# jeff-regier/Celeste.jl

Hardware: AMD Instinct MI355X
Metric: sources/sec (ELBO value+gradient+Hessian+KL per target source) (higher is better)
Workload: dtype f64; 1 GPU; BASELINE.json configs[2]: synthetic 2048x1489x5 SDSS-size field, 2000 star+galaxy sources, fp64, Sa=1 with value-only neighbours, psf_K=2; gather_backend=none, neighbor_links_rank0=3526

## Files before the change

### celeste.jl_amd/csrc/celeste_abi.hip

```cpp
#include <hip/hip_runtime.h>
#include <algorithm>
#include <atomic>
#include <cmath>
#include <cstdio>
#include <cstdlib>
#include <cstring>
#include <mutex>
#include <unordered_map>
#include <vector>

#include "elbo_kernels.h"
#include "optim_kernels.h"
#include "fused_kernels.h"
#include "host_tables.h"

struct celeste_group;

#define EVAL_FUSED_MAX 32

#define HIP_TRY(expr)                                                                    \
    do {                                                                                 \
        hipError_t e__ = (expr);                                                         \
        if (e__ != hipSuccess) {                                                         \
            fprintf(stderr, "celeste_mi355x: %s failed: %s (%s:%d)\n", #expr,            \
// ... 50 lines not shown
    return cap;
}
static hipError_t staging_alloc(void **p, size_t bytes) {
    *p = nullptr;
    int k = -1;
    if (pinned_pool_cap() && bytes <= (1u << 20)) { k = 0; while (((size_t)4096 << k) < bytes) ++k; }
    if (k < 0) return hipHostMalloc(p, std::max<size_t>(bytes, 1), hipHostMallocPortable);
    PinnedPool &pp = pinned_pool();
    {
        std::lock_guard<std::mutex> lk(pp.mu);
        if (!pp.idle[k].empty()) { *p = pp.idle[k].back(); pp.idle[k].pop_back(); pp.idle_bytes -= (size_t)4096 << k; pp.live[*p] = k; return hipSuccess; }
    }
    hipError_t e = hipHostMalloc(p, (size_t)4096 << k, hipHostMallocPortable);
    if (e == hipSuccess) { std::lock_guard<std::mutex> lk(pp.mu); pp.live[*p] = k; }
    return e;
}
static void staging_free(void *p) {
    if (!p) return;
    {
        PinnedPool &pp = pinned_pool();
        std::lock_guard<std::mutex> lk(pp.mu);
        auto it = pp.live.find(p);
        if (it != pp.live.end()) {
            const int k = it->second;
            pp.live.erase(it);
            if (pp.idle_bytes + ((size_t)4096 << k) <= pinned_pool_cap()) { pp.idle[k].push_back(p); pp.idle_bytes += (size_t)4096 << k; return; }
        }
    }
    (void)hipHostFree(p);
}


struct celeste_images {
    int device = 0;
    int N = 0;
    std::vector<DevImage> h_images;
    std::vector<void *> plane_allocs;
    DevImage *d_images = nullptr;
    std::atomic<int> refs{1};
};

static void images_release(celeste_images *im) {
    if (!im || im->refs.fetch_sub(1) != 1) return;
    (void)hipSetDevice(im->device);
    for (void *p : im->plane_allocs) (void)hipFree(p);
    if (im->d_images) (void)hipFree(im->d_images);
    delete im;
}

struct celeste_ctx {
    int device = 0;
    celeste_images *imgs = nullptr;
    hipStream_t stream = nullptr;
    hipStream_t copy_stream = nullptr;
    bool copy_stream_checked = false;
    int N = 0, S = 0, K = 0, NC = 0, n_stamps = 0;
    int chunk_px = 256, CH = 1;
    int max_npx = 0;
    std::vector<DevPatch> h_patches;
    std::vector<int64_t> h_nbr_off;
    std::vector<int32_t> h_nbr_idx;
    DevImage *d_images = nullptr;
    DevPatch *d_patches = nullptr;
    double *d_coefs = nullptr;
    float *d_coefs_f = nullptr;
    uint8_t *d_bitmaps = nullptr;
    int64_t *d_nbr_off = nullptr;
    int32_t *d_nbr_idx = nullptr;
    PriorDev *d_prior = nullptr;
    SrcImg *d_srcimg = nullptr;
    Comp *d_comps = nullptr;
    SrcGeo *d_geo = nullptr;
    int64_t *d_val_off = nullptr;
    double2 *d_val = nullptr;
    int32_t *d_needed = nullptr;
    int32_t stamp = 0;
    std::vector<int32_t> h_vis_off, h_vis_img, h_vis_src;
    int32_t *d_vis_off = nullptr, *d_vis_img = nullptr, *d_vis_src = nullptr;
    int4 *d_value_items = nullptr;
    int4 *d_vitems_src = nullptr;
    int32_t *d_vitem_off = nullptr;
    std::vector<int32_t> h_vitem_off;
    int64_t n_value_items = 0;
    int32_t *d_prep_mark = nullptr;
    double *d_lg_sum = nullptr;
    int64_t *d_nv_base = nullptr;
    int32_t *d_nbr_vis = nullptr;
    int2 *d_items = nullptr;
    size_t items_cap = 0;
    std::vector<int32_t> h_src_chunks;
    std::vector<int64_t> h_top_chunks;
    int max_src_chunks = 0;
    int32_t *d_work = nullptr, *d_work_blk = nullptr, *d_work_total = nullptr;
    size_t work_cap = 0, work_blk_cap = 0;
    int M = 1;
    bool dense = false;
    int64_t V = 0;
    std::vector<int64_t> h_tile_off;
    int64_t *d_tile_off = nullptr;
    int64_t n_tiles = 0;
    int sum_tiles = 4, RCH = 1;
    double *d_rec = nullptr;
    double *d_acc_split = nullptr;
    size_t acc_split_cap = 0;
    double *d_acc = nullptr;
    size_t acc_cap = 0;
    int32_t *d_rec_off = nullptr;
    size_t rec_off_cap = 0;
    double *d_vp = nullptr;
    int32_t *d_targets = nullptr;
    double *d_v = nullptr, *d_d = nullptr, *d_h = nullptr;
    int64_t *d_cnt = nullptr;
    int32_t *d_status = nullptr;
    size_t stage_cap = 0;
    double *p_vp = nullptr;
    int32_t *p_targets = nullptr, *p_status = nullptr;
    double *p_v = nullptr, *p_d = nullptr, *p_h = nullptr;
    int64_t *p_cnt = nullptr;
    size_t pin_cap = 0;
    double *d_small_in = nullptr, *p_small_in = nullptr, *d_small_out = nullptr, *p_small_out = nullptr;
    static const int MAX_PARTS = 8;
    hipEvent_t part_done[MAX_PARTS] = {}, part_copied[MAX_PARTS] = {};
    struct OptBuffers {
        size_t cap = 0;
        double *d_vp = nullptr, *d_v = nullptr, *d_d = nullptr, *d_h = nullptr, *d_H = nullptr, *d_T = nullptr, *d_S = nullptr, *d_pos = nullptr;
        int32_t *d_targets = nullptr, *d_act[2] = {nullptr, nullptr}, *d_evt[2] = {nullptr, nullptr}, *d_count = nullptr,
                *d_st = nullptr;
        void *d_state = nullptr;
        static const int RING = 4;
        double *h_vp = nullptr;
        void *h_state = nullptr;
        int32_t *h_count = nullptr;
        hipEvent_t ev[RING] = {};
    } opt;
    struct FusedBuffers {
        size_t cap_t = 0, cap_rec = 0, cap_q = 0, cap_saved = 0;
        bool arrivals_dirty = true;
        int4 *d_chunk_desc = nullptr;
        int2 *d_tgt_rec = nullptr;
        int32_t *d_q_items = nullptr, *d_q_ctl = nullptr, *d_arrivals = nullptr;
        double *d_saved = nullptr;
        int32_t *h_ctl = nullptr;
        int max_resident = 0;
        int cus = 0;
    } fused;
    struct Scratch { void *p = nullptr; size_t cap = 0; } scratch[24];
    int timing = 0;
    hipEvent_t ev[5] = {nullptr, nullptr, nullptr, nullptr, nullptr};
    int ev_split = 0;
    int ev_valid = 0;
};

#define ABI_CATCH catch (const std::bad_alloc &) { return CELESTE_ERR_ALLOC; } catch (...) { return CELESTE_ERR_HIP; }

extern "C" int celeste_version(void) { return CELESTE_ABI_VERSION; }

extern "C" const char *celeste_strerror(int status) {
    switch (status) {
        case CELESTE_OK: return "ok";
        case CELESTE_ERR_INVALID_ARG: return "invalid argument";
        case CELESTE_ERR_NONFINITE_INPUT: return "vp contains NaNs or Infs";
        case CELESTE_ERR_NONFINITE_RESULT: return "ELBO value, gradient or Hessian contains Inf/NaNs";
        case CELESTE_ERR_HIP: return "HIP runtime error";
        case CELESTE_ERR_NO_DEVICE: return "no HIP device (the engine has no CPU fallback)";
        case CELESTE_ERR_ALLOC: return "allocation failed";
        case CELESTE_ERR_ABORTED: return "device group aborted: a member failed in front of a collective (destroy the group and create it again)";
// ... 249 lines not shown
        PriorDev pd;
        pd.p = pr->prior ? *pr->prior : DEFAULT_PRIOR;
        for (int i = 0; i < 2; ++i) for (int d = 0; d < 8; ++d) inv4_logdet(pd.p.color_cov[i][d], pd.inv_cov[i][d], &pd.logdet[i][d]);
        CTX_TRY(dev_upload(&c->d_prior, &pd, 1));
    }
    {
        static std::mutex consts_mu;
        static bool consts_ready[16] = {};
        std::lock_guard<std::mutex> lk(consts_mu);
        if (device < 0 || device >= 16 || !consts_ready[device]) {
            double eta[16], nu[16];
            galaxy_prototypes(eta, nu);
            if (hipMemcpyToSymbol(HIP_SYMBOL(c_eta), eta, sizeof eta) != hipSuccess ||
                hipMemcpyToSymbol(HIP_SYMBOL(c_nu), nu, sizeof nu) != hipSuccess) {
                celeste_ctx_destroy(c); return CELESTE_ERR_HIP;
            }
            hipLaunchKernelGGL(exp_table_kernel, dim3(1), dim3(64), 0, nullptr);
            if (hipStreamSynchronize(nullptr) != hipSuccess) { celeste_ctx_destroy(c); return CELESTE_ERR_HIP; }
            if (device >= 0 && device < 16) consts_ready[device] = true;
        }
    }
    CTX_TRY(dev_upload<SrcImg>(&c->d_srcimg, nullptr, (size_t)c->V));
    CTX_TRY(dev_upload<Comp>(&c->d_comps, nullptr, (size_t)c->V * c->NC));
    CTX_TRY(dev_upload<SrcGeo>(&c->d_geo, nullptr, (size_t)c->S));
    {
        std::vector<int64_t> voff(c->h_patches.size());
        int64_t tot = 0;
        for (size_t q = 0; q < c->h_patches.size(); ++q) { voff[q] = tot; tot += (int64_t)c->h_patches[q].H2 * c->h_patches[q].W2; }
        CTX_TRY(dev_upload(&c->d_val_off, voff.data(), voff.size()));
        CTX_TRY(dev_upload<double2>(&c->d_val, nullptr, (size_t)tot));
        CTX_TRY(dev_upload<int32_t>(&c->d_needed, nullptr, (size_t)c->S));
        if (hipMemset(c->d_needed, 0, (size_t)c->S * sizeof(int32_t)) != hipSuccess) { celeste_ctx_destroy(c); return CELESTE_ERR_HIP; }
    }

    CTX_TRY(dev_upload(&c->d_vis_off, c->h_vis_off.data(), c->h_vis_off.size()));
    CTX_TRY(dev_upload(&c->d_vis_img, c->h_vis_img.data(), c->h_vis_img.size()));
    CTX_TRY(dev_upload(&c->d_vis_src, c->h_vis_src.data(), c->h_vis_src.size()));
    CTX_TRY(dev_upload<double>(&c->d_lg_sum, nullptr, (size_t)c->V));
    if (c->V > 0)
        hipLaunchKernelGGL(patch_lgamma_kernel, dim3((unsigned)c->V), dim3(256), 0, nullptr, c->d_images, c->d_patches,
                           c->d_vis_img, c->d_bitmaps, c->d_lg_sum);
    const char *env_chunk = getenv("CELESTE_CHUNK_PX");
    if (env_chunk && atoi(env_chunk) >= 64) c->chunk_px = (atoi(env_chunk) + 63) / 64 * 64;
    c->CH = c->max_npx > 0 ? (c->max_npx + c->chunk_px - 1) / c->chunk_px : 1;
    c->h_src_chunks.assign((size_t)c->S, 0);
    for (int s = 0; s < c->S; ++s) {
        for (int v = c->h_vis_off[s]; v < c->h_vis_off[s + 1]; ++v) {
            const DevPatch &q = c->h_patches[v];
            c->h_src_chunks[s] += (q.H2 * q.W2 + c->chunk_px - 1) / c->chunk_px;
        }
        c->max_src_chunks = std::max(c->max_src_chunks, c->h_src_chunks[s]);
    }
    auto hv = [c](int s, int n) -> int64_t {
        if (c->dense) return (int64_t)s * c->N + n;
        const int32_t *b = c->h_vis_img.data() + c->h_vis_off[s], *e = c->h_vis_img.data() + c->h_vis_off[s + 1];
        const int32_t *it = std::lower_bound(b, e, n);
        return it != e && *it == n ? (int64_t)(it - c->h_vis_img.data()) : -1;
    };
    if (!c->dense) {
        std::vector<int64_t> base((size_t)c->S + 1, 0);
        for (int s = 0; s < c->S; ++s)
            base[s + 1] = base[s] + (int64_t)(c->h_vis_off[s + 1] - c->h_vis_off[s]) * (c->h_nbr_off[s + 1] - c->h_nbr_off[s]);
        std::vector<int32_t> nv((size_t)base[c->S]);
        for (int s = 0; s < c->S; ++s) {
            const int64_t K = c->h_nbr_off[s + 1] - c->h_nbr_off[s];
            for (int v = c->h_vis_off[s]; v < c->h_vis_off[s + 1]; ++v)
                for (int64_t q = 0; q < K; ++q)
                    nv[base[s] + (int64_t)(v - c->h_vis_off[s]) * K + q] = (int32_t)hv(c->h_nbr_idx[c->h_nbr_off[s] + q], c->h_vis_img[v]);
        }
        CTX_TRY(dev_upload(&c->d_nv_base, base.data(), base.size()));
        CTX_TRY(dev_upload(&c->d_nbr_vis, nv.data(), nv.size()));
    }
    {
        std::vector<int32_t> sorted(c->h_src_chunks);
        std::sort(sorted.begin(), sorted.end(), [](int32_t a, int32_t b) { return a > b; });
        c->h_top_chunks.assign((size_t)c->S + 1, 0);
        for (int s = 0; s < c->S; ++s) c->h_top_chunks[s + 1] = c->h_top_chunks[s] + sorted[s];
    }
    CTX_TRY(dev_upload<int32_t>(&c->d_work_total, nullptr, 1));
    {
        if (c->N > 0xffff) { celeste_ctx_destroy(c); return CELESTE_ERR_INVALID_ARG; }
        const int n_cls = c->chunk_px / 64;
        std::vector<std::vector<std::pair<int32_t, int32_t>>> by_len(n_cls);
        for (int s = 0; s < c->S; ++s)
            for (int64_t q = c->h_nbr_off[s]; q < c->h_nbr_off[s + 1]; ++q) {
                const int s2 = c->h_nbr_idx[q];
                for (int va = c->h_vis_off[s]; va < c->h_vis_off[s + 1]; ++va) {
                    const int n = c->h_vis_img[va];
                    const int64_t vb = hv(s2, n);
                    if (vb < 0) continue;
                    const DevPatch &a = c->h_patches[va], &b = c->h_patches[vb];
                    const int rh = std::min(a.off_h + a.H2, b.off_h + b.H2) - std::max(a.off_h, b.off_h);
                    const int rw = std::min(a.off_w + a.W2, b.off_w + b.W2 - 1) - std::max(a.off_w, b.off_w);
                    if (rh <= 0 || rw <= 0) continue;
                    const int npx = rh * rw, nch = (npx + c->chunk_px - 1) / c->chunk_px;
                    for (int ch = 0; ch < nch; ++ch) {
                        const int px = std::min(c->chunk_px, npx - ch * c->chunk_px);
                        by_len[n_cls - (px + 63) / 64].push_back({(int32_t)q, (int32_t)(n | (ch << 16))});
                    }
                }
            }
        std::vector<int32_t> link_src(c->h_nbr_idx.size());
        for (int s = 0; s < c->S; ++s)
            for (int64_t q = c->h_nbr_off[s]; q < c->h_nbr_off[s + 1]; ++q) link_src[q] = s;
        std::vector<int4> desc;
        for (auto &v : by_len)
            for (auto &e : v) {
                const int t = link_src[e.first], s2 = c->h_nbr_idx[e.first], n = e.second & 0xffff, ch = e.second >> 16;
                desc.push_back(make_int4((int)hv(s2, n), (int)hv(t, n), ch, t));
            }
        c->n_value_items = (int64_t)desc.size();
        CTX_TRY(dev_upload(&c->d_value_items, desc.data(), desc.size()));
        c->h_vitem_off.assign((size_t)c->S + 1, 0);
        for (auto &d : desc) c->h_vitem_off[(size_t)d.w + 1]++;
        for (int s = 0; s < c->S; ++s) c->h_vitem_off[s + 1] += c->h_vitem_off[s];
        {
            std::vector<int4> by_src(desc.size());
            std::vector<int32_t> fill(c->h_vitem_off.begin(), c->h_vitem_off.end() - 1);
            for (auto &d : desc) by_src[(size_t)fill[d.w]++] = d;
            CTX_TRY(dev_upload(&c->d_vitems_src, by_src.data(), by_src.size()));
            CTX_TRY(dev_upload(&c->d_vitem_off, c->h_vitem_off.data(), c->h_vitem_off.size()));
        }
        CTX_TRY(dev_upload<int32_t>(&c->d_prep_mark, nullptr, (size_t)c->S));
        if (hipMemset(c->d_prep_mark, 0, (size_t)c->S * sizeof(int32_t)) != hipSuccess) { celeste_ctx_destroy(c); return CELESTE_ERR_HIP; }
    }
    {
        c->h_tile_off.resize(c->h_patches.size());
        int64_t tot = 0;
        for (size_t q = 0; q < c->h_patches.size(); ++q) {
            c->h_tile_off[q] = tot;
            tot += ((int64_t)c->h_patches[q].H2 * c->h_patches[q].W2 + 63) / 64;
        }
        c->n_tiles = tot;
        if (const char *e = getenv("CELESTE_SUM_TILES")) if (atoi(e) > 0) c->sum_tiles = atoi(e);
        c->RCH = std::max(1, ((c->max_npx + 63) / 64 + c->sum_tiles - 1) / c->sum_tiles);
    }
    if (hipStreamSynchronize(nullptr) != hipSuccess) { celeste_ctx_destroy(c); return CELESTE_ERR_HIP; }
#undef CTX_TRY
    *out = c;
    return CELESTE_OK;
} ABI_CATCH

extern "C" void celeste_ctx_destroy(celeste_ctx_t *c) {
    if (!c) return;
    (void)hipSetDevice(c->device);
    if (c->stream) (void)hipStreamSynchronize(c->stream);
    if (c->copy_stream) (void)hipStreamSynchronize(c->copy_stream);
    void *ptrs[] = {c->d_patches, c->d_coefs, c->d_coefs_f, c->d_bitmaps, c->d_nbr_off, c->d_nbr_idx, c->d_prior,
                    c->d_srcimg, c->d_comps, c->d_geo, c->d_val_off, c->d_val, c->d_needed, c->d_vis_off, c->d_vis_img, c->d_vis_src, c->d_value_items, c->d_vitems_src, c->d_vitem_off, c->d_prep_mark, c->d_rec_off, c->d_lg_sum, c->d_nv_base, c->d_nbr_vis, c->d_items, c->d_work, c->d_work_blk, c->d_work_total, c->d_tile_off, c->d_rec, c->d_acc_split, c->d_acc, c->d_vp, c->d_targets, c->d_v, c->d_d, c->d_h,
                    c->d_cnt, c->d_status};
    for (void *p : ptrs) if (p) (void)hipFree(p);
    {
        auto &o = c->opt;
        void *optr[] = {o.d_vp, o.d_v, o.d_d, o.d_h, o.d_H, o.d_T, o.d_S, o.d_pos, o.d_targets, o.d_act[0], o.d_act[1], o.d_evt[0], o.d_evt[1],
                        o.d_count, o.d_st, o.d_state};
        for (void *q : optr) if (q) (void)hipFree(q);
        void *hptr[] = {o.h_vp, o.h_state, o.h_count};
        for (void *q : hptr) if (q) staging_free(q);
        for (int k = 0; k < celeste_ctx::OptBuffers::RING; ++k) if (o.ev[k]) (void)hipEventDestroy(o.ev[k]);
        auto &f = c->fused;
        void *fptr[] = {f.d_chunk_desc, f.d_tgt_rec, f.d_q_items, f.d_q_ctl, f.d_arrivals, f.d_saved};
        for (void *q : fptr) if (q) (void)hipFree(q);
        if (f.h_ctl) staging_free(f.h_ctl);
    }
    for (auto &sc : c->scratch) if (sc.p) (void)hipFree(sc.p);
    for (int i = 0; i < 5; ++i) if (c->ev[i]) (void)hipEventDestroy(c->ev[i]);
    for (int i = 0; i < celeste_ctx::MAX_PARTS; ++i) {
        if (c->part_done[i]) (void)hipEventDestroy(c->part_done[i]);
        if (c->part_copied[i]) (void)hipEventDestroy(c->part_copied[i]);
    }
    void *pins[] = {c->p_vp, c->p_targets, c->p_status, c->p_v, c->p_d, c->p_h, c->p_cnt, c->p_small_in, c->p_small_out};
    if (c->d_small_in) (void)hipFree(c->d_small_in);
    if (c->d_small_out) (void)hipFree(c->d_small_out);
    for (void *q : pins) if (q) staging_free(q);
    stream_retire(c->device, c->stream);
    stream_retire(c->device, c->copy_stream);
    images_release(c->imgs);
    delete c;
}

template <class T>
static hipError_t scratch_get(celeste_ctx_t *c, int k, size_t bytes, T **out) {
    auto &s = c->scratch[k];
    if (bytes > s.cap) {
        hipError_t e = s.p ? hipStreamSynchronize(c->stream) : hipSuccess;
        if (e != hipSuccess) return e;
        if (s.p) { (void)hipFree(s.p); s.p = nullptr; s.cap = 0; }
        e = hipMalloc(&s.p, std::max<size_t>(bytes, 256));
        if (e != hipSuccess) return e;
        s.cap = std::max<size_t>(bytes, 256);
    }
    *out = (T *)s.p;
    return hipSuccess;
}

static int launch_eval(celeste_ctx_t *c, const double *d_vp, int32_t n_targets, const int32_t *d_targets,
                       uint32_t flags, double *d_v, double *d_d, double *d_h, int64_t *d_counters, int32_t *d_status,
                       void *stream_, bool render_neighbors, const int32_t *d_active_rank = nullptr,
                       int64_t n_chunks = -1, bool tables_current = false, const int32_t *d_live = nullptr,
                       bool prep_all = false, bool render_only = false, const int32_t *d_h_pos = nullptr);

extern "C" int celeste_elbo_eval_batch_device(celeste_ctx_t *c, const double *d_vp, int32_t n_targets,
                                              const int32_t *d_targets, uint32_t flags, double *d_v, double *d_d,
                                              double *d_h, int64_t *d_counters, int32_t *d_status, void *stream_) try {
    return launch_eval(c, d_vp, n_targets, d_targets, flags, d_v, d_d, d_h, d_counters, d_status, stream_, true);
} ABI_CATCH

static int ensure_part_events(celeste_ctx_t *c, int n) {
    for (int k = 0; k < n && k < celeste_ctx::MAX_PARTS; ++k) {
        if (!c->part_done[k]) HIP_TRY(hipEventCreateWithFlags(&c->part_done[k], hipEventDisableTiming));
        if (!c->part_copied[k]) HIP_TRY(hipEventCreateWithFlags(&c->part_copied[k], hipEventDisableTiming));
    }
    return CELESTE_OK;
}

static void fused_args_tables(celeste_ctx_t *c, FusedArgs &A) {
    A.images = c->d_images; A.patches = c->d_patches; A.coefs = c->d_coefs; A.bitmaps = c->d_bitmaps;
    A.nbr_off = c->d_nbr_off; A.nbr_idx = c->d_nbr_idx; A.val_off = c->d_val_off; A.val = c->d_val;
    A.nv_base = c->d_nv_base; A.nbr_vis = c->d_nbr_vis; A.items = c->dense ? nullptr : c->d_items; A.geo = c->d_geo;
    A.prior = c->d_prior; A.vis_off = c->d_vis_off; A.vis_img = c->d_vis_img; A.lg_sum = c->d_lg_sum; A.rec_off = c->d_rec_off;
    A.N = c->N; A.NC = c->NC; A.K = c->K; A.M = c->M; A.CH = c->CH; A.chunk_px = c->chunk_px;
    A.acc = c->d_acc;
    A.st = nullptr; A.Hstate = nullptr; A.Tstate = nullptr; A.Spec = nullptr; A.q_items = nullptr; A.q_ctl = nullptr; A.q_cap = 0; A.timeout_ticks = 0;
    A.j_R = 0; A.j_gshift = 0; A.j_dep = nullptr; A.j_succ_off = nullptr; A.j_succ = nullptr; A.j_vitem_off = nullptr;
    A.j_vitems = nullptr; A.j_render_arr = nullptr; A.j_saved = nullptr; A.j_pos = nullptr; A.j_srcimg = nullptr;
    A.j_comps = nullptr; A.j_geo = nullptr;
}

static int fused_buffers(celeste_ctx_t *c, size_t n, size_t rec, hipStream_t stream) {
    auto &fb = c->fused;
    if (n > fb.cap_t) {
        if (fb.d_tgt_rec || fb.d_arrivals) HIP_TRY(hipStreamSynchronize(stream));
// ... 70 lines not shown
    if (eval_fused) G = 1;
    const int n_classes = WORK_CLASSES;
    if ((size_t)n_wblk * (n_classes + 1) > c->work_blk_cap) {
        if (c->d_work_blk) { HIP_TRY(hipStreamSynchronize(stream)); HIP_TRY(hipFree(c->d_work_blk)); c->d_work_blk = nullptr; }
        HIP_TRY(hipMalloc((void **)&c->d_work_blk, (size_t)n_wblk * (n_classes + 1) * sizeof(int32_t)));
        c->work_blk_cap = (size_t)n_wblk * (n_classes + 1);
    }
    const bool derivs = (flags & (CELESTE_FLAG_GRAD | CELESTE_FLAG_HESS)) != 0;
    const bool split = (flags & CELESTE_FLAG_SPLIT) != 0;
    if (split) {
        if (!(flags & CELESTE_FLAG_HESS)) return CELESTE_ERR_INVALID_ARG;
        if (!c->d_rec) {
            HIP_TRY(hipStreamSynchronize(stream));
            if (dev_upload(&c->d_tile_off, c->h_tile_off.data(), c->h_tile_off.size()) != CELESTE_OK) return CELESTE_ERR_HIP;
            if (hipMalloc((void **)&c->d_rec, (size_t)std::max<int64_t>(c->n_tiles, 1) * ACC_N * 64 * sizeof(double)) != hipSuccess)
                return CELESTE_ERR_ALLOC;
        }
        const size_t need_s = (size_t)n_targets * c->M * c->RCH * ACC_N;
        if (need_s > c->acc_split_cap) {
            if (c->d_acc_split) { HIP_TRY(hipStreamSynchronize(stream)); HIP_TRY(hipFree(c->d_acc_split)); c->d_acc_split = nullptr; }
            HIP_TRY(hipMalloc((void **)&c->d_acc_split, need_s * sizeof(double)));
            c->acc_split_cap = need_s;
        }
    }
    if (c->timing) HIP_TRY(hipEventRecord(c->ev[0], stream));
    if (render_neighbors && ++c->stamp == 0x7fffffff) {
        HIP_TRY(hipMemsetAsync(c->d_needed, 0, (size_t)c->S * sizeof(int32_t), stream));
        c->stamp = 1;
    }
    const int geo_S = render_neighbors ? c->S : -1;
    const size_t setup_threads = std::max<size_t>(render_neighbors ? (size_t)c->S : 0, (size_t)n_targets * (c->dense ? 1 : c->M));
    int32_t *const prep_mark = render_neighbors && !tables_current && !prep_all ? c->d_prep_mark : nullptr;
    bool prep_fused = false;
    bool records_described = false;
    if (eval_fused) { int stb = fused_buffers(c, (size_t)n_targets, rec_cap, stream); if (stb != CELESTE_OK) return stb; }
    if (n_visits <= WORK1_MAX_VISITS && !getenv("CELESTE_PARALLEL_WORKLIST")) {
        const unsigned setup_blocks = (unsigned)((setup_threads + WORK1_SETUP - 1) / WORK1_SETUP);
        prep_fused = !render_neighbors && !getenv("CELESTE_NO_FUSED_PREP");
        const bool prep_all_here = render_neighbors && !tables_current && c->V > 0 && c->V <= WORK1_PREP_ALL_MAX &&
                                   (n_targets >= WORK1_PREP_ALL_MIN_TARGETS || c->V <= WORK1_PREP_ALL_TINY) && !getenv("CELESTE_NO_FUSED_PREP");
        const int prep_n = prep_all_here ? (int)c->V : n_visits;
        if (prep_all_here) prep_fused = true;
        const unsigned prep_blocks = prep_fused ? (unsigned)((prep_n + WORK1_NT / 64 - 1) / (WORK1_NT / 64)) : 0u;
        const bool records_described_here = eval_fused && c->dense && !d_live && !getenv("CELESTE_NO_FUSED_DESCRIBE");
        hipLaunchKernelGGL(setup_worklist_kernel, dim3(1 + setup_blocks + prep_blocks), dim3(WORK1_NT),
                           0, stream, d_vp, geo_S, c->d_geo, d_targets, n_targets, c->d_vis_off, c->d_vis_img, c->M,
                           c->dense ? nullptr : c->d_items, render_neighbors ? c->d_needed : nullptr, c->stamp, c->d_patches,
                           c->N, CH, chunk_px, G, (int)c->dense, c->d_work, c->d_work_total, d_live, prep_mark,
                           c->d_nbr_off, c->d_nbr_idx, c->d_rec_off, (int)setup_blocks, c->d_images, c->K, c->d_srcimg,
                           c->d_comps, prep_all_here ? (int)c->V : 0, c->d_vis_src,
                           records_described_here ? c->fused.d_chunk_desc : nullptr, records_described_here ? c->fused.d_tgt_rec : nullptr,
                           c->chunk_px);
        records_described = records_described_here;
    } else {
        hipLaunchKernelGGL(setup_kernel, dim3((unsigned)((setup_threads + 63) / 64)), dim3(64), 0, stream, d_vp, geo_S,
                           c->d_geo, d_targets, n_targets, c->d_vis_off, c->d_vis_img, c->M, c->dense ? nullptr : c->d_items,
                           render_neighbors ? c->d_needed : nullptr, c->stamp, prep_mark, c->d_nbr_off, c->d_nbr_idx, d_live);
        hipLaunchKernelGGL(work_count_kernel, dim3(n_wblk), dim3(WORK_NT), 0, stream, d_targets, n_visits, c->d_patches,
                           c->d_vis_off, c->d_vis_img, c->N, c->M, chunk_px, G, (int)c->dense, c->d_work_blk, d_live);
        hipLaunchKernelGGL(work_scan_kernel, dim3(1), dim3(1024), 0, stream, c->d_work_blk, n_wblk * (n_classes + 1),
                           c->d_work_total, n_wblk * n_classes);
        hipLaunchKernelGGL(work_fill_kernel, dim3(n_wblk), dim3(WORK_NT), 0, stream, d_targets, n_visits, c->d_patches,
                           c->d_vis_off, c->d_vis_img, c->N, c->M, CH, chunk_px, G, (int)c->dense, c->d_work_blk, c->d_work, d_live,
                           c->d_rec_off);
    }
    if (render_neighbors) {
        if (c->V > 0 && !tables_current && !prep_fused)
            hipLaunchKernelGGL(prep_kernel, dim3((unsigned)c->V), dim3(64), 0, stream, d_vp, c->d_images, c->d_patches,
                               c->d_vis_src, c->d_vis_img, c->N, c->K, c->d_srcimg, c->d_comps, nullptr, c->d_vis_off, c->M,
                               (int)c->dense, nullptr, prep_mark, c->stamp);
    } else if (!prep_fused) {
        hipLaunchKernelGGL(prep_kernel, dim3((unsigned)std::max(n_visits, 1)), dim3(64), 0, stream, d_vp, c->d_images,
                           c->d_patches, c->d_vis_src, c->d_vis_img, c->N, c->K, c->d_srcimg, c->d_comps, d_targets,
                           c->d_vis_off, c->M, (int)c->dense, d_live, nullptr, 0);
    }
    if (render_neighbors) {
    if (c->n_value_items > 0)
    {
        const bool wide_items = n_targets <= VALUE_WIDE_MAX && c->chunk_px == 256 && !getenv("CELESTE_NO_WIDE_VALUE");
#define LAUNCH_VALUE(R, WAVES)                                                                                              \
        hipLaunchKernelGGL((value_kernel<R, WAVES>), dim3((unsigned)c->n_value_items), dim3(64 * WAVES), 0, stream,       \
                           c->d_patches, c->d_coefs, c->d_srcimg, c->d_comps, c->d_needed, c->stamp, c->d_val_off,          \
                           c->d_value_items, c->NC, c->chunk_px, c->d_val, c->d_coefs_f)
        if (flags & CELESTE_FLAG_FP32) { if (wide_items) LAUNCH_VALUE(float, 2); else LAUNCH_VALUE(float, 1); }
        else { if (wide_items) LAUNCH_VALUE(double, 4); else LAUNCH_VALUE(double, 1); }
#undef LAUNCH_VALUE
    }
    }
    if (render_only) { HIP_TRY(hipGetLastError()); return CELESTE_OK; }
    if (c->timing) HIP_TRY(hipEventRecord(c->ev[1], stream));
    if (eval_fused) {
        auto &fb = c->fused;
        if (fb.arrivals_dirty) {
            HIP_TRY(hipMemsetAsync(fb.d_arrivals, 0, fb.cap_t * sizeof(int32_t), stream));
            fb.arrivals_dirty = false;
        }
        if (!records_described)
            hipLaunchKernelGGL(fused_setup_kernel, dim3((unsigned)((n_targets + 63) / 64)), dim3(64), 0, stream, d_targets, n_targets,
                               c->d_patches, c->d_vis_off, c->dense ? nullptr : c->d_items, c->N, c->M, c->chunk_px, c->d_rec_off,
                               fb.d_chunk_desc, fb.d_tgt_rec, (int32_t *)nullptr, (int32_t *)nullptr);
        FusedArgs A;
        fused_args_tables(c, A);
        A.targets = d_targets; A.n_targets = n_targets; A.vp = const_cast<double *>(d_vp);
        A.chunk_desc = fb.d_chunk_desc; A.tgt_rec = fb.d_tgt_rec; A.arrivals = fb.d_arrivals; A.flags = flags;
        memset(&A.op, 0, sizeof A.op);
        const unsigned rec_bound = (unsigned)std::max<size_t>(n_chunks >= 0 ? grid_need : work_need, 1);
        hipLaunchKernelGGL(eval_fused_kernel, dim3(rec_bound + (unsigned)n_targets), dim3(FUSED_NT), 0, stream, A, c->d_srcimg,
                           c->d_comps, c->d_work_total, (int)rec_bound, d_v, d_d, d_h, d_counters, d_status);
        if (c->timing) { HIP_TRY(hipEventRecord(c->ev[2], stream)); HIP_TRY(hipEventRecord(c->ev[3], stream)); c->ev_valid = 1; c->ev_split = 0; }
        HIP_TRY(hipGetLastError());
        return CELESTE_OK;
    }
    const dim3 grid((unsigned)std::max<size_t>(grid_need, 1));
#define PIXEL_ARGS                                                                                                \
    c->d_images, c->d_patches, c->d_coefs, c->d_bitmaps, c->d_srcimg, c->d_comps, c->d_nbr_off, c->d_nbr_idx,       \
    c->d_val_off, c->d_val, d_targets, c->N, c->NC, CH, chunk_px, G, c->d_acc, c->d_tile_off, c->d_rec, \
    d_active_rank, c->d_items, c->M, c->d_work, c->d_work_total, c->d_nv_base, c->d_nbr_vis, c->d_rec_off, c->d_coefs_f
#define LAUNCH_PIXEL_T(MODE, R) hipLaunchKernelGGL((pixel_kernel<MODE, R>), grid, dim3(64), 0, stream, PIXEL_ARGS)
#define LAUNCH_PIXEL_M(MODE) hipLaunchKernelGGL((pixel_kernel<MODE, double, true>), grid, dim3(64), 0, stream, PIXEL_ARGS)
#define LAUNCH_PIXEL(MODE) do { if (flags & CELESTE_FLAG_FP32) LAUNCH_PIXEL_T(MODE, float); else LAUNCH_PIXEL_T(MODE, double); } while (0)
    if (d_active_rank) {
        if (flags & CELESTE_FLAG_HESS) LAUNCH_PIXEL_M(2);
        else if (derivs) LAUNCH_PIXEL_M(1);
        else LAUNCH_PIXEL_M(0);
    }
    else if (split) LAUNCH_PIXEL(3);
    else if (flags & CELESTE_FLAG_HESS) LAUNCH_PIXEL(2);
    else if (derivs) LAUNCH_PIXEL(1);
    else LAUNCH_PIXEL_T(0, double);
#undef LAUNCH_PIXEL
#undef LAUNCH_PIXEL_M
#undef PIXEL_ARGS
#undef LAUNCH_PIXEL_T
    if (c->timing) HIP_TRY(hipEventRecord(c->ev[2], stream));
    c->ev_split = 0;
    const int lift_nt = n_targets <= 1024 ? 512 : 256;
    bool lift7 = n_targets > 4096;
    if (const char *e = getenv("CELESTE_LIFT_WAVES")) lift7 = atoi(e) == 7;
#define LAUNCH_LIFT(...) do { if (lift7) hipLaunchKernelGGL(lift_kernel<7>, __VA_ARGS__); else hipLaunchKernelGGL(lift_kernel<8>, __VA_ARGS__); } while (0)
    if (split) {
        hipLaunchKernelGGL(record_sum_kernel, dim3((unsigned)((size_t)n_targets * c->M * c->RCH)), dim3(RSUM_NT), 0,
                           stream, c->d_patches, d_targets, c->d_tile_off, reinterpret_cast<const double2 *>(c->d_rec),
                           c->d_items, c->N, c->M, c->RCH, c->sum_tiles, c->d_acc_split, nullptr, c->d_work_total);
        if (c->timing) { HIP_TRY(hipEventRecord(c->ev[4], stream)); c->ev_split = 1; }
        LAUNCH_LIFT(dim3(n_targets), dim3(lift_nt), 0, stream, d_vp, c->d_images, c->d_patches, c->d_geo,
                           c->d_nbr_off, c->d_nbr_idx, d_targets, c->d_acc_split, c->d_prior, c->d_vis_off, c->d_vis_img, c->N, c->M,
                           c->RCH, c->sum_tiles * 64, flags,
                           d_v, d_d, d_h, d_counters, d_status, d_live, d_active_rank ? nullptr : c->d_lg_sum, nullptr, d_h_pos);
    } else
    LAUNCH_LIFT(dim3(n_targets), dim3(lift_nt), 0, stream, d_vp, c->d_images, c->d_patches, c->d_geo,
                       c->d_nbr_off, c->d_nbr_idx, d_targets, c->d_acc, c->d_prior, c->d_vis_off, c->d_vis_img, c->N, c->M, CH,
                       chunk_px, flags,
                       d_v, d_d, d_h, d_counters, d_status, d_live, d_active_rank ? nullptr : c->d_lg_sum, c->d_rec_off, d_h_pos);
#undef LAUNCH_LIFT
    if (c->timing) { HIP_TRY(hipEventRecord(c->ev[3], stream)); c->ev_valid = 1; }
    HIP_TRY(hipGetLastError());
    return CELESTE_OK;
}

__global__ void spin_kernel(long long ticks) {
    const long long t0 = wall_clock64();
    while (wall_clock64() - t0 < ticks) __builtin_amdgcn_s_sleep(8);
}
static int pick_copy_stream(celeste_ctx_t *c) {
    if (c->copy_stream_checked) return CELESTE_OK;
    c->copy_stream_checked = true;
    if (const char *e = getenv("CELESTE_COPY_STREAM_CHECK")) if (atoi(e) == 0) return CELESTE_OK;
    const size_t bytes = 4u << 20;
// ... 1035 lines not shown
```

### celeste.jl_amd/csrc/elbo_kernels.h

```cpp
#pragma once
#include <hip/hip_runtime.h>
#include <math.h>
#include "elbo_device.h"
#include "../../include/celeste_mi355x.h"

#ifndef CELESTE_MUTANT
#define CELESTE_MUTANT 0
#endif

__constant__ double c_eta[16];
__constant__ double c_nu[16];

__device__ inline void bvn_cov(double ab, double angle, double scale, double &x11, double &x12, double &x22) {
    double sp, cp;
    sincos(angle, &sp, &cp);
    double ab_term = ab * ab - 1.0;
    double s2 = scale * scale;
    x12 = -s2 * cp * sp * ab_term;
    x11 = s2 * (1.0 + ab_term * (sp * sp));
    x22 = s2 * (1.0 + ab_term * (cp * cp));
}

__device__ inline void brightness(const double *vs, int i, int b, double &El, double &Ell) {
    const double r = vs[6 + i], v = vs[8 + i];
// ... 662 lines not shown
            if (k < prep_all_V) prep_visit(threadIdx.x & 63, vis_src[k], vis_img[k], k, vp, images, patches, K, srcimg, comps);
            return;
        }
        const int ti = k / M, j = k - ti * M;
        if (ti >= n_targets || (live && ti >= *live)) return;
        const int s = targets[ti];
        int n = j;
        if (!dense) {
            const int vo = vis_off[s];
            if (j >= vis_off[s + 1] - vo) return;
            n = vis_img[vo + j];
        }
        const int sn = dense ? s * N + n : vis_off[s] + j;
        const DevPatch &q = patches[sn];
        if (q.H2 * q.W2 <= 0) return;
        prep_visit(threadIdx.x & 63, s, n, sn, vp, images, patches, K, srcimg, comps);
        return;
    }
    if (blockIdx.x > 0) {
        if (threadIdx.x < WORK1_SETUP)
            setup_thread((blockIdx.x - 1) * WORK1_SETUP + threadIdx.x, vp, S, geo, targets, n_targets, vis_off, vis_img, M,
                         items, is_target, stamp, prep_mark, nbr_off, nbr_idx, live);
        return;
    }
    __shared__ int s_part[WORK1_NT / 64];
    __shared__ int s_base[WORK_CLASSES + 2];
    int n_visits = n_targets * M;
    if (live) n_visits = min(n_visits, *live * M);
    const int per = (n_visits + WORK1_NT - 1) / WORK1_NT;
    const int k0 = threadIdx.x * per, k1 = min(n_visits, k0 + per);
    const int lane = threadIdx.x & 63, wv = threadIdx.x >> 6;
    constexpr int NCL = WORK_CLASSES + 1;
    int cnt[NCL];
#pragma unroll
    for (int c = 0; c < NCL; ++c) cnt[c] = 0;
    for (int k = k0; k < k1; ++k) {
        int n_full, lc, nch;
        visit_chunks(k, targets, patches, vis_off, vis_img, N, M, chunk_px, G, dense != 0, n_full, lc, &nch);
        cnt[0] += n_full;
#pragma unroll
        for (int c = 1; c < WORK_CLASSES; ++c) cnt[c] += lc == c;
        cnt[WORK_CLASSES] += nch;
    }
    int off[NCL];
    if (threadIdx.x == 0) s_base[0] = 0;
#pragma unroll
    for (int c = 0; c < NCL; ++c) {
        int x = cnt[c];
#pragma unroll
        for (int d = 1; d < 64; d <<= 1) { const int y = __shfl_up(x, d); if (lane >= d) x += y; }
        __syncthreads();
        if (lane == 63) s_part[wv] = x;
        __syncthreads();
        int before = 0, tot = 0;
#pragma unroll
        for (int w = 0; w < WORK1_NT / 64; ++w) { const int v = s_part[w]; before += w < wv ? v : 0; tot += v; }
        off[c] = before + x - cnt[c];
        if (threadIdx.x == 0) s_base[c + 1] = s_base[c] + tot;
    }
    __syncthreads();
    if (threadIdx.x == 0) *work_total = s_base[WORK_CLASSES];
#pragma unroll
    for (int c = 0; c < WORK_CLASSES; ++c) off[c] += s_base[c];
    for (int k = k0; k < k1; ++k) {
        int n_full, lc, nch;
        visit_chunks(k, targets, patches, vis_off, vis_img, N, M, chunk_px, G, dense != 0, n_full, lc, &nch);
        for (int g = 0; g < n_full; ++g) work[off[0]++] = k * CH + g * G;
#pragma unroll
        for (int c = 1; c < WORK_CLASSES; ++c) if (lc == c) work[off[c]++] = k * CH + n_full * G;
        rec_off[k] = off[WORK_CLASSES];
        off[WORK_CLASSES] += nch;
    }
    if (fz_tgt_rec) {
        __syncthreads();
        for (int ti = threadIdx.x; ti < n_targets; ti += WORK1_NT) {
            int first;
            const int n_rec = describe_target_records(ti, targets[ti], patches, nullptr, N, M, fz_chunk_px, rec_off, fz_chunk_desc, first);
            fz_tgt_rec[ti] = make_int2(first < 0 ? 0 : first, n_rec);
        }
    }
}

template <bool COH, typename R = double>
__device__ __forceinline__ void value_pixels(int lane, const DevPatch &P, const SrcImg &si, const Comp *__restrict__ tc, int NC,
                                             const double *__restrict__ coefs, const double *__restrict__ etab, int h_lo,
                                             int w_lo, int RH, int p0, int p1, double2 *__restrict__ out,
                                             const float *__restrict__ tcf = nullptr) {
    const double *__restrict__ coef = coefs + (size_t)(CELESTE_MUTANT == 3 ? 0 : P.stamp) * (CEL_COEF * CEL_COEF);
    const double sh0 = 26.0 - si.m1, sw0 = 26.0 - si.m2;
    const float rRH = 1.0f / (float)RH;
    for (int idx = p0 + lane; idx < p1; idx += 64) {
        int rw, rh;
        divmod_small(idx, RH, rRH, rw, rh);
        const int h0 = h_lo + rh, w0 = w_lo + rw;
        const double hh = (double)(h0 + 1), ww = (double)(w0 + 1);
        double f0, f1;
        if constexpr (sizeof(R) == 8) {
            f0 = star_value(coef, hh + sh0, ww + sw0);
            f1 = galaxy_value(tc, NC, hh - si.m1, ww - si.m2, etab);
        } else {
            f0 = (double)star_value_f(coef, (float)(hh + sh0), (float)(ww + sw0));
            f1 = (double)galaxy_value_f(tcf, NC, (float)(hh - si.m1), (float)(ww - si.m2));
        }
        const double En = si.c0 * f0 + si.c1 * f1;
        const double E2n = si.q0 * (f0 * f0) + si.q1 * (f1 * f1);
        double2 *const o = out + ((h0 - P.off_h) + (int64_t)P.H2 * (w0 - P.off_w));
        const double var = E2n - En * En;
        if constexpr (COH) { stc<true>(&o->x, En); stc<true>(&o->y, var); }
        else *o = make_double2(En, var);
    }
}

typedef float f2v __attribute__((ext_vector_type(2)));
__device__ __forceinline__ void value_pixels_f2(int lane, const DevPatch &P, const SrcImg &si, int NC, const float *__restrict__ coef,
                                                int h_lo, int w_lo, int RH, int p0, int p1, double2 *__restrict__ out,
                                                const float *__restrict__ tcf) {
    const double sh0 = 26.0 - si.m1, sw0 = 26.0 - si.m2;
    const float rRH = 1.0f / (float)RH;
    const f2v *tp = reinterpret_cast<const f2v *>(tcf);
    const int n_dev = 8 * (NC / 14);
    for (int base = p0; base < p1; base += 128) {
        int h0[2], w0[2];
        bool ok[2];
        float dxs[2], dys[2], xh[2], xw[2];
#pragma unroll
        for (int q = 0; q < 2; ++q) {
            const int i = base + 64 * q + lane;
            ok[q] = i < p1;
            int rw, rh;
            divmod_small(min(i, p1 - 1), RH, rRH, rw, rh);
            h0[q] = h_lo + rh; w0[q] = w_lo + rw;
            const double hh = (double)(h0[q] + 1), ww = (double)(w0[q] + 1);
            dxs[q] = (float)(hh - si.m1); dys[q] = (float)(ww - si.m2);
            xh[q] = (float)(hh + sh0); xw[q] = (float)(ww + sw0);
        }
        const f2v dx = {dxs[0], dxs[1]}, dy = {dys[0], dys[1]};
        f2v f1 = (f2v)(0.0f);
        for (int c0 = 0; c0 < NC; c0 += (c0 < n_dev ? 8 : 6)) {
            const int len = c0 < n_dev ? 8 : 6;
            const f2v *k0 = tp + 3 * c0;
            const f2v d1 = dx - k0[3].xx, d2 = dy - k0[4].xx;
            const f2v s11 = -0.72134752044448170368f * (d1 * d1), s12 = -1.44269504088896340736f * (d1 * d2),
                      s22 = -0.72134752044448170368f * (d2 * d2);
            for (int c = c0; c < c0 + len; c += 2) {
                const f2v *k = tp + 3 * c;
                {
                    const f2v p11 = k[0].xx, p12 = k[1].xx, p22 = k[2].xx, w = k[5].xx;
                    const f2v q2 = p11 * s11 + (p12 * s12 + p22 * s22);
                    f1 += w * (f2v){__builtin_amdgcn_exp2f(q2.x), __builtin_amdgcn_exp2f(q2.y)};
                }
                {
#if CELESTE_MUTANT == 6
                    const f2v p11 = k[0].yy, p12 = k[1].xx, p22 = k[2].yy, w = k[5].yy;
#else
                    const f2v p11 = k[0].yy, p12 = k[1].yy, p22 = k[2].yy, w = k[5].yy;
#endif
                    const f2v q2 = p11 * s11 + (p12 * s12 + p22 * s22);
                    f1 += w * (f2v){__builtin_amdgcn_exp2f(q2.x), __builtin_amdgcn_exp2f(q2.y)};
                }
            }
        }
        const float *cc[2];
        float fxs[2], fys[2];
#pragma unroll
        for (int q = 0; q < 2; ++q) {
            int ix = (int)floorf(xh[q]); ix = ix < 1 ? 1 : (ix > 50 ? 50 : ix);
            int iy = (int)floorf(xw[q]); iy = iy < 1 ? 1 : (iy > 50 ? 50 : iy);
            cc[q] = coef + (ix - 1) + CEL_COEF * (iy - 1);
            fxs[q] = xh[q] - (float)ix; fys[q] = xw[q] - (float)iy;
        }
        f2v wx[4], wy[4];
        bspline_w((f2v){fxs[0], fxs[1]}, wx); bspline_w((f2v){fys[0], fys[1]}, wy);
        f2v y = (f2v)(0.0f);
#pragma unroll
        for (int b = 0; b < 4; ++b) {
            const float *ca = cc[0] + CEL_COEF * b, *cb = cc[1] + CEL_COEF * b;
            const f2v r = (f2v){ca[0], cb[0]} * wx[0] + (f2v){ca[1], cb[1]} * wx[1] + (f2v){ca[2], cb[2]} * wx[2] + (f2v){ca[3], cb[3]} * wx[3];
            y += r * wy[b];
        }
        const float f0s[2] = {y.x < 0 ? 1e-3f * __expf(y.x) : 1e-3f * (y.x + 1.0f), y.y < 0 ? 1e-3f * __expf(y.y) : 1e-3f * (y.y + 1.0f)};
        const float f1s[2] = {f1.x, f1.y};
#pragma unroll
        for (int q = 0; q < 2; ++q) {
            if (!ok[q]) continue;
            const double f0 = (double)f0s[q], g1 = (double)f1s[q];
            const double En = si.c0 * f0 + si.c1 * g1;
            const double E2n = si.q0 * (f0 * f0) + si.q1 * (g1 * g1);
            out[(h0[q] - P.off_h) + (int64_t)P.H2 * (w0[q] - P.off_w)] = make_double2(En, E2n - En * En);
        }
    }
}

#ifdef VALUE_TIMING
__device__ unsigned long long g_value_clk[8];
#endif
template <typename R, int WAVES = 1>
__global__ void __launch_bounds__(64 * WAVES)
value_kernel(const DevPatch *__restrict__ patches, const double *__restrict__ coefs,
             const SrcImg *__restrict__ srcimg, const Comp *__restrict__ comps,
             const int32_t *__restrict__ is_target, int32_t stamp, const int64_t *__restrict__ val_off,
             const int4 *__restrict__ items, int NC, int chunk_px, double2 *__restrict__ val,
             const float *__restrict__ coefs_f) {
    __shared__ double etab[64];
#ifdef VALUE_TIMING
    long long vts[4]; vts[0] = clock64();
#define VT(k) do { vts[(k) + 1] = clock64(); } while (0)
#else
#define VT(k) do { } while (0)
#endif
    const int4 it = items[blockIdx.x];
    const int sn = it.x, ch = it.z, t = it.w;
    if (is_target[t] != stamp) return;
    const DevPatch &P = patches[sn];
    const DevPatch &T = patches[it.y];
    const int h_lo = max(P.off_h, T.off_h), h_hi = min(P.off_h + P.H2, T.off_h + T.H2);
    const int w_lo = max(P.off_w, T.off_w), w_hi = min(P.off_w + P.W2 - 1, T.off_w + T.W2);
    const int RH = h_hi - h_lo, RW = w_hi - w_lo;
    if (RH <= 0 || RW <= 0) return;
    const int npx = RH * RW;
    const int p0 = ch * chunk_px;
    if (p0 >= npx) return;
    VT(0);
    exp_table_init(etab);
    const int p1 = min(npx, p0 + chunk_px);
    const SrcImg si = srcimg[sn];
    __shared__ Comp tc[14 * CEL_MAXK];
    {
        const double *src = reinterpret_cast<const double *>(comps + (size_t)sn * NC);
        double *dst = reinterpret_cast<double *>(tc);
        for (int i = threadIdx.x; i < NC * 8; i += 64 * WAVES) dst[i] = src[i];
        __syncthreads();
    }
    __shared__ float tcf[sizeof(R) == 4 ? 6 * 14 * CEL_MAXK : 2];
    if constexpr (sizeof(R) == 4) {
        if ((int)threadIdx.x < NC) {
            const Comp k = tc[threadIdx.x];
            float *o = tcf + 12 * (threadIdx.x >> 1) + (threadIdx.x & 1);
            o[0] = (float)k.p11; o[2] = (float)k.p12; o[4] = (float)k.p22; o[6] = (float)k.xi1; o[8] = (float)k.xi2; o[10] = (float)k.w0;
        }
        __syncthreads();
    }
    VT(1);
    if constexpr (sizeof(R) == 4) {
        const int q0 = p0 + 128 * (int)(threadIdx.x >> 6);
        if (WAVES == 1 || q0 < p1)
            value_pixels_f2(threadIdx.x & 63, P, si, NC, coefs_f + (size_t)(CELESTE_MUTANT == 3 ? 0 : P.stamp) * (CEL_COEF * CEL_COEF), h_lo, w_lo, RH,
                            WAVES == 1 ? p0 : q0, WAVES == 1 ? p1 : min(p1, q0 + 128), val + val_off[sn], tcf);
    } else if constexpr (WAVES == 1)
        value_pixels<false, R>(threadIdx.x, P, si, tc, NC, coefs, etab, h_lo, w_lo, RH, p0, p1, val + val_off[sn], tcf);
    else {
        const int q0 = p0 + 64 * (int)(threadIdx.x >> 6);
        if (q0 < p1) value_pixels<false, R>(threadIdx.x & 63, P, si, tc, NC, coefs, etab, h_lo, w_lo, RH, q0, min(p1, q0 + 64), val + val_off[sn], tcf);
    }
    VT(2);
#ifdef VALUE_TIMING
    if (threadIdx.x == 0) {
        for (int k = 0; k < 3; ++k) atomicAdd(&g_value_clk[k], (unsigned long long)(vts[k + 1] - vts[k]));
        atomicAdd(&g_value_clk[7], 1ull); atomicAdd(&g_value_clk[6], (unsigned long long)((p1 - p0 + 63) / 64));
    }
#endif
#undef VT
}

template <typename S>
struct PixelTermsT {
    typedef S scalar;
    S vterm, cnt_act, cnt_inact;
    S f0, f1;
    S alpha, beta, w2, w12;
    S k0, k1;
    S f0g0, f0g1, f0h0, f0h1, f0h2;
    S C0s, C0g, C1s, C1g;
    S Q0s, Q0g, Q1s, Q1g;
    S Wgg, Wsg, Wss;
    S S0d, S1x, S1y, S1xd, S1yd, S2a, S2b, S2c, S2an, S2bn, S2cn, S2ad, S2bd, S2cd;
    S S3a, S3b, S3c, S3d, S4a, S4b, S4c, S4d, S4e;
};
typedef PixelTermsT<double> PixelTerms;

template <int G, class TT>
__device__ __forceinline__ typename TT::scalar gal_g(const TT &T) {
    typedef typename TT::scalar S;
    if constexpr (G == 0) return T.S1x;
    else if constexpr (G == 1) return T.S1y;
    else if constexpr (G == 2) return T.S0d;
    else if constexpr (G == 3) return (S)0.5 * T.S2an;
    else if constexpr (G == 4) return T.S2bn;
    else return (S)0.5 * T.S2cn;
}
template <int G, int G2, class TT>
__device__ __forceinline__ typename TT::scalar gal_h(const TT &T) {
    typedef typename TT::scalar S;
    constexpr int k = G * 6 + G2;
    if constexpr (k == 0) return T.S2a;
    else if constexpr (k == 1) return T.S2b;
    else if constexpr (k == 2) return T.S1xd;
    else if constexpr (k == 3) return (S)0.5 * T.S3a;
    else if constexpr (k == 4) return T.S3b;
    else if constexpr (k == 5) return (S)0.5 * T.S3c;
    else if constexpr (k == 7) return T.S2c;
    else if constexpr (k == 8) return T.S1yd;
    else if constexpr (k == 9) return (S)0.5 * T.S3b;
    else if constexpr (k == 10) return T.S3c;
    else if constexpr (k == 11) return (S)0.5 * T.S3d;
    else if constexpr (k == 14) return (S)0.0;
    else if constexpr (k == 15) return (S)0.5 * T.S2ad;
    else if constexpr (k == 16) return T.S2bd;
    else if constexpr (k == 17) return (S)0.5 * T.S2cd;
    else if constexpr (k == 21) return (S)0.25 * T.S4a;
    else if constexpr (k == 22) return (S)0.5 * T.S4b;
    else if constexpr (k == 23) return (S)0.25 * T.S4c;
    else if constexpr (k == 28) return T.S4c;
    else if constexpr (k == 29) return (S)0.5 * T.S4d;
    else { static_assert(k == 35, "upper triangle only"); return (S)0.25 * T.S4e; }
}
template <int G, class TT>
__device__ __forceinline__ typename TT::scalar star_g(const TT &T) {
    typedef typename TT::scalar S;
    if constexpr (G == 0) return T.f0g0;
    else if constexpr (G == 1) return T.f0g1;
    else return (S)0.0;
}
constexpr int hess_row(int e) {
    int i = 0, k = e - ACC_H0;
    while (k >= ZV - i) { k -= ZV - i; ++i; }
    return i;
}
constexpr int hess_col(int e) {
    int i = 0, k = e - ACC_H0;
    while (k >= ZV - i) { k -= ZV - i; ++i; }
    return i + k;
}

template <int E, class TT>
__device__ __forceinline__ typename TT::scalar record_entry(const TT &T) {
    typedef typename TT::scalar S;
    if constexpr (E == 0) return T.vterm;
    else if constexpr (E == ACC_CNT) return T.cnt_act;
    else if constexpr (E == ACC_CNT + 1) return T.cnt_inact;
    else if constexpr (E <= ZV) {
        constexpr int r = E - 1;
        if constexpr (r == 0) return T.alpha * T.f0;
        else if constexpr (r == 1) return T.alpha * T.f1;
        else if constexpr (r == 2) return T.w2 * T.f0 * T.f0;
// ... 1779 lines not shown
```

Measured before the change: 3.088 million sources/sec.

## Compute neighbour values per patch over deduplicated pixel units

Adds a value_unit_kernel that evaluates each neighbour patch's value/variance once over the union of the pixels its target links overlap. The old scheme issued one work item per (link, chunk), so a pixel shared by several links was computed more than once. At context creation the host builds a per-patch pixel list, splits it into fixed-size units, and sorts the units by size. Each block exits early if none of its linked targets are active. This fp64 non-wide path is now the default, while the old kernel remains behind an environment variable. It costs extra setup work and an indirect pixel-index load for each pixel.

```diff
diff --git a/celeste.jl_amd/csrc/celeste_abi.hip b/celeste.jl_amd/csrc/celeste_abi.hip
--- a/celeste.jl_amd/csrc/celeste_abi.hip
+++ b/celeste.jl_amd/csrc/celeste_abi.hip
@@ -156,6 +156,10 @@
     int32_t *d_vitem_off = nullptr;
     std::vector<int32_t> h_vitem_off;
     int64_t n_value_items = 0;
+    int4 *d_vunit_items = nullptr;
+    int32_t *d_vunit_lnk_off = nullptr, *d_vunit_lnk = nullptr;
+    int32_t *d_vunit_px = nullptr;
+    int64_t n_vunit_items = 0;
     int32_t *d_prep_mark = nullptr;
     double *d_lg_sum = nullptr;
     int64_t *d_nv_base = nullptr;
@@ -571,6 +575,7 @@
         if (c->N > 0xffff) { celeste_ctx_destroy(c); return CELESTE_ERR_INVALID_ARG; }
         const int n_cls = c->chunk_px / 64;
         std::vector<std::vector<std::pair<int32_t, int32_t>>> by_len(n_cls);
+        std::vector<std::vector<std::pair<int32_t, int4>>> by_unit(c->h_patches.size());
         for (int s = 0; s < c->S; ++s)
             for (int64_t q = c->h_nbr_off[s]; q < c->h_nbr_off[s + 1]; ++q) {
                 const int s2 = c->h_nbr_idx[q];
@@ -582,6 +587,8 @@
                     const int rh = std::min(a.off_h + a.H2, b.off_h + b.H2) - std::max(a.off_h, b.off_h);
                     const int rw = std::min(a.off_w + a.W2, b.off_w + b.W2 - 1) - std::max(a.off_w, b.off_w);
                     if (rh <= 0 || rw <= 0) continue;
+                    by_unit[(size_t)vb].push_back({(int32_t)s, make_int4(std::max(a.off_h, b.off_h) - b.off_h,
+                                                                         std::max(a.off_w, b.off_w) - b.off_w, rh, rw)});
                     const int npx = rh * rw, nch = (npx + c->chunk_px - 1) / c->chunk_px;
                     for (int ch = 0; ch < nch; ++ch) {
                         const int px = std::min(c->chunk_px, npx - ch * c->chunk_px);
@@ -610,6 +617,45 @@
             CTX_TRY(dev_upload(&c->d_vitems_src, by_src.data(), by_src.size()));
             CTX_TRY(dev_upload(&c->d_vitem_off, c->h_vitem_off.data(), c->h_vitem_off.size()));
         }
+        {
+            int unit_px = VALUE_UNIT_PX;
+            if (const char *e = getenv("CELESTE_VALUE_UNIT_PX")) if (atoi(e) >= 1) unit_px = (atoi(e) + VALUE_UNIT_NT - 1) / VALUE_UNIT_NT * VALUE_UNIT_NT;
+            std::vector<int32_t> lnk_off(c->h_patches.size() + 1, 0), lnk, px;
+            std::vector<std::vector<int4>> by_pass(unit_px / VALUE_UNIT_NT);
+            std::vector<uint8_t> mark;
+            for (size_t vb = 0; vb < by_unit.size(); ++vb) {
+                const auto &u = by_unit[vb];
+                lnk_off[vb + 1] = lnk_off[vb] + (int32_t)u.size();
+                if (u.empty()) continue;
+                const DevPatch &b = c->h_patches[vb];
+                if (b.H2 > 0xffff || b.W2 > 0x7fff) { celeste_ctx_destroy(c); return CELESTE_ERR_INVALID_ARG; }
+                mark.assign((size_t)b.H2 * b.W2, 0);
+                for (const auto &e : u) {
+                    lnk.push_back(e.first);
+                    const int4 r = e.second;
+                    for (int w = r.y; w < r.y + r.w; ++w) memset(&mark[(size_t)r.x + (size_t)b.H2 * w], 1, (size_t)r.z);
+                }
+                const int64_t p0 = (int64_t)px.size();
+                for (int w = 0; w < b.W2; ++w)
+                    for (int h = 0; h < b.H2; ++h)
+                        if (mark[(size_t)h + (size_t)b.H2 * w]) px.push_back(h | (w << 16));
+                const int64_t p1 = (int64_t)px.size();
+                if (p1 > 0x7fffffff) { celeste_ctx_destroy(c); return CELESTE_ERR_INVALID_ARG; }
+                for (int64_t q = p0; q < p1; q += unit_px) {
+                    const int n = (int)std::min<int64_t>(unit_px, p1 - q);
+                    by_pass[(n + VALUE_UNIT_NT - 1) / VALUE_UNIT_NT - 1].push_back(make_int4((int)vb, (int)q, (int)(q + n), 0));
+                }
+            }
+            std::vector<int4> uitems;
+            for (int k = (int)by_pass.size() - 1; k >= 0; --k) uitems.insert(uitems.end(), by_pass[k].begin(), by_pass[k].end());
+            c->n_vunit_items = (int64_t)uitems.size();
+            if (!uitems.empty()) {
+                CTX_TRY(dev_upload(&c->d_vunit_items, uitems.data(), uitems.size()));
+                CTX_TRY(dev_upload(&c->d_vunit_lnk_off, lnk_off.data(), lnk_off.size()));
+                CTX_TRY(dev_upload(&c->d_vunit_lnk, lnk.data(), lnk.size()));
+                CTX_TRY(dev_upload(&c->d_vunit_px, px.data(), px.size()));
+            }
+        }
         CTX_TRY(dev_upload<int32_t>(&c->d_prep_mark, nullptr, (size_t)c->S));
         if (hipMemset(c->d_prep_mark, 0, (size_t)c->S * sizeof(int32_t)) != hipSuccess) { celeste_ctx_destroy(c); return CELESTE_ERR_HIP; }
     }
@@ -636,7 +682,7 @@
     if (c->stream) (void)hipStreamSynchronize(c->stream);
     if (c->copy_stream) (void)hipStreamSynchronize(c->copy_stream);
     void *ptrs[] = {c->d_patches, c->d_coefs, c->d_coefs_f, c->d_bitmaps, c->d_nbr_off, c->d_nbr_idx, c->d_prior,
-                    c->d_srcimg, c->d_comps, c->d_geo, c->d_val_off, c->d_val, c->d_needed, c->d_vis_off, c->d_vis_img, c->d_vis_src, c->d_value_items, c->d_vitems_src, c->d_vitem_off, c->d_prep_mark, c->d_rec_off, c->d_lg_sum, c->d_nv_base, c->d_nbr_vis, c->d_items, c->d_work, c->d_work_blk, c->d_work_total, c->d_tile_off, c->d_rec, c->d_acc_split, c->d_acc, c->d_vp, c->d_targets, c->d_v, c->d_d, c->d_h,
+                    c->d_srcimg, c->d_comps, c->d_geo, c->d_val_off, c->d_val, c->d_needed, c->d_vis_off, c->d_vis_img, c->d_vis_src, c->d_value_items, c->d_vitems_src, c->d_vitem_off, c->d_vunit_items, c->d_vunit_lnk_off, c->d_vunit_lnk, c->d_vunit_px, c->d_prep_mark, c->d_rec_off, c->d_lg_sum, c->d_nv_base, c->d_nbr_vis, c->d_items, c->d_work, c->d_work_blk, c->d_work_total, c->d_tile_off, c->d_rec, c->d_acc_split, c->d_acc, c->d_vp, c->d_targets, c->d_v, c->d_d, c->d_h,
                     c->d_cnt, c->d_status};
     for (void *p : ptrs) if (p) (void)hipFree(p);
     {
@@ -873,8 +919,14 @@
         hipLaunchKernelGGL((value_kernel<R, WAVES>), dim3((unsigned)c->n_value_items), dim3(64 * WAVES), 0, stream,       \
                            c->d_patches, c->d_coefs, c->d_srcimg, c->d_comps, c->d_needed, c->stamp, c->d_val_off,          \
                            c->d_value_items, c->NC, c->chunk_px, c->d_val, c->d_coefs_f)
+        const bool units = !wide_items && c->n_vunit_items > 0 && !getenv("CELESTE_NO_VALUE_UNITS");
         if (flags & CELESTE_FLAG_FP32) { if (wide_items) LAUNCH_VALUE(float, 2); else LAUNCH_VALUE(float, 1); }
-        else { if (wide_items) LAUNCH_VALUE(double, 4); else LAUNCH_VALUE(double, 1); }
+        else if (wide_items) LAUNCH_VALUE(double, 4);
+        else if (units)
+            hipLaunchKernelGGL(value_unit_kernel, dim3((unsigned)c->n_vunit_items), dim3(VALUE_UNIT_NT), 0, stream, c->d_patches,
+                               c->d_coefs, c->d_srcimg, c->d_comps, c->d_needed, c->stamp, c->d_val_off, c->d_vunit_items,
+                               c->d_vunit_lnk_off, c->d_vunit_lnk, c->d_vunit_px, c->NC, c->d_val);
+        else LAUNCH_VALUE(double, 1);
 #undef LAUNCH_VALUE
     }
     }
diff --git a/celeste.jl_amd/csrc/elbo_kernels.h b/celeste.jl_amd/csrc/elbo_kernels.h
--- a/celeste.jl_amd/csrc/elbo_kernels.h
+++ b/celeste.jl_amd/csrc/elbo_kernels.h
@@ -768,6 +768,27 @@
 }
 
 template <bool COH, typename R = double>
+__device__ __forceinline__ void value_pixel(const DevPatch &P, const SrcImg &si, const Comp *__restrict__ tc, int NC,
+                                            const double *__restrict__ coef, const double *__restrict__ etab, double sh0,
+                                            double sw0, int h0, int w0, double2 *__restrict__ out, const float *__restrict__ tcf) {
+    const double hh = (double)(h0 + 1), ww = (double)(w0 + 1);
+    double f0, f1;
+    if constexpr (sizeof(R) == 8) {
+        f0 = star_value(coef, hh + sh0, ww + sw0);
+        f1 = galaxy_value(tc, NC, hh - si.m1, ww - si.m2, etab);
+    } else {
+        f0 = (double)star_value_f(coef, (float)(hh + sh0), (float)(ww + sw0));
+        f1 = (double)galaxy_value_f(tcf, NC, (float)(hh - si.m1), (float)(ww - si.m2));
+    }
+    const double En = si.c0 * f0 + si.c1 * f1;
+    const double E2n = si.q0 * (f0 * f0) + si.q1 * (f1 * f1);
+    double2 *const o = out + ((h0 - P.off_h) + (int64_t)P.H2 * (w0 - P.off_w));
+    const double var = E2n - En * En;
+    if constexpr (COH) { stc<true>(&o->x, En); stc<true>(&o->y, var); }
+    else *o = make_double2(En, var);
+}
+
+template <bool COH, typename R = double>
 __device__ __forceinline__ void value_pixels(int lane, const DevPatch &P, const SrcImg &si, const Comp *__restrict__ tc, int NC,
                                              const double *__restrict__ coefs, const double *__restrict__ etab, int h_lo,
                                              int w_lo, int RH, int p0, int p1, double2 *__restrict__ out,
@@ -778,22 +799,7 @@
     for (int idx = p0 + lane; idx < p1; idx += 64) {
         int rw, rh;
         divmod_small(idx, RH, rRH, rw, rh);
-        const int h0 = h_lo + rh, w0 = w_lo + rw;
-        const double hh = (double)(h0 + 1), ww = (double)(w0 + 1);
-        double f0, f1;
-        if constexpr (sizeof(R) == 8) {
-            f0 = star_value(coef, hh + sh0, ww + sw0);
-            f1 = galaxy_value(tc, NC, hh - si.m1, ww - si.m2, etab);
-        } else {
-            f0 = (double)star_value_f(coef, (float)(hh + sh0), (float)(ww + sw0));
-            f1 = (double)galaxy_value_f(tcf, NC, (float)(hh - si.m1), (float)(ww - si.m2));
-        }
-        const double En = si.c0 * f0 + si.c1 * f1;
-        const double E2n = si.q0 * (f0 * f0) + si.q1 * (f1 * f1);
-        double2 *const o = out + ((h0 - P.off_h) + (int64_t)P.H2 * (w0 - P.off_w));
-        const double var = E2n - En * En;
-        if constexpr (COH) { stc<true>(&o->x, En); stc<true>(&o->y, var); }
-        else *o = make_double2(En, var);
+        value_pixel<COH, R>(P, si, tc, NC, coef, etab, sh0, sw0, h_lo + rh, w_lo + rw, out, tcf);
     }
 }
 
@@ -946,6 +952,42 @@
     }
 #endif
 #undef VT
+}
+
+#define VALUE_UNIT_NT 256
+#define VALUE_UNIT_PX 1024
+__global__ void __launch_bounds__(VALUE_UNIT_NT)
+value_unit_kernel(const DevPatch *__restrict__ patches, const double *__restrict__ coefs, const SrcImg *__restrict__ srcimg,
+                  const Comp *__restrict__ comps, const int32_t *__restrict__ is_target, int32_t stamp,
+                  const int64_t *__restrict__ val_off, const int4 *__restrict__ items ,
+                  const int32_t *__restrict__ lnk_off , const int32_t *__restrict__ lnk, const int32_t *__restrict__ px,
+                  int NC, double2 *__restrict__ val) {
+    __shared__ double etab[64];
+    __shared__ Comp tc[14 * CEL_MAXK];
+    const int4 it = items[blockIdx.x];
+    const int sn = it.x;
+    {
+        const int lane = threadIdx.x & 63;
+        bool any = false;
+        for (int q = lnk_off[sn] + lane; q < lnk_off[sn + 1]; q += 64) any |= is_target[lnk[q]] == stamp;
+        if (__ballot(any) == 0ull) return;
+    }
+    exp_table_init(etab);
+    {
+        const double *src = reinterpret_cast<const double *>(comps + (size_t)sn * NC);
+        double *dst = reinterpret_cast<double *>(tc);
+        for (int i = threadIdx.x; i < NC * 8; i += VALUE_UNIT_NT) dst[i] = src[i];
+        __syncthreads();
+    }
+    const DevPatch &P = patches[sn];
+    const SrcImg si = srcimg[sn];
+    const double *__restrict__ coef = coefs + (size_t)(CELESTE_MUTANT == 3 ? 0 : P.stamp) * (CEL_COEF * CEL_COEF);
+    const double sh0 = 26.0 - si.m1, sw0 = 26.0 - si.m2;
+    double2 *const out = val + val_off[sn];
+    for (int i = it.y + (int)threadIdx.x; i < it.z; i += VALUE_UNIT_NT) {
+        const int e = px[i];
+        value_pixel<false, double>(P, si, tc, NC, coef, etab, sh0, sw0, P.off_h + (e & 0xffff), P.off_w + (e >> 16), out, nullptr);
+    }
 }
 
 template <typename S>
```

Result: faster. 3.129 million sources/sec, median of 6 (+1.3%).
